# phecda-xu/FullyCNNSpeechEnhancement

Hardware: AMD Instinct MI355X
Metric: spectrogram frames/sec (CR-CED-16 fwd, 129-bin) (higher is better)
Workload: dtype f32; 1 GPU; CR-CED V3 (16-layer, skip connections) forward, batch 256 per GPU, 129x512, fp32 (BASELINE configs[2]); variant=FullyCNNV3, batch_per_gpu=256, frames=512, bins=129, global_batch=256, fused_available=True, parallelism=batch-shard x1, rccl_world_size=1, weights=random-init (glorot, seed 42), library=rced-hip 0.1 gfx950

## Files before the change

fullycnnspeechenhancement_amd/csrc/kernels_fused_v3.h:

```cpp
#pragma once
#include <hip/hip_runtime.h>

#include <type_traits>

#include "lds_dma.h"

#ifndef RCED_V3_LEGACY_FORMS
#define RCED_V3_LEGACY_FORMS 0
#endif
#ifndef RCED_D1
#define RCED_D1 1
#endif
#ifndef RCED_D2
#define RCED_D2 2
#endif
#ifndef RCED_D2X
#define RCED_D2X 1
#endif
#ifndef RCED_D3
#define RCED_D3 2
#endif
#ifndef RCED_LANE_OPAQUE
#define RCED_LANE_OPAQUE 1
#endif
#ifndef RCED_L1_ORDER
#define RCED_L1_ORDER 1
#endif
#ifndef RCED_L3_CHAINS
#define RCED_L3_CHAINS 2
#endif
#ifndef RCED_L2_BOTH
#define RCED_L2_BOTH 1
#endif
#ifndef RCED_T_L1X6
#define RCED_T_L1X6 1
#endif
#ifndef RCED_T_L1SWAP
#define RCED_T_L1SWAP 1
#endif
#ifndef RCED_V3_LB
#define RCED_V3_LB kThreads
#endif
#ifndef RCED_STAMPS
#define RCED_STAMPS 0
#endif

namespace rced {
namespace v3 {

#if RCED_STAMPS
__device__ __forceinline__ unsigned long long stamp() {
  unsigned long long t;
  __builtin_amdgcn_sched_barrier(0);
  asm volatile("s_memtime %0\n\ts_waitcnt lgkmcnt(0)" : "=s"(t)::"memory");
  __builtin_amdgcn_sched_barrier(0);
  return t;
}
#define STAMP_BEGIN() const unsigned long long st_a_ = stamp()
#define STAMP_MATH(i) const unsigned long long st_b_ = stamp(); tsum[i] += st_b_ - st_a_
#define STAMP_WAIT(i) tsum[(i) + ((i) < 3 ? 3 : 1)] += stamp() - st_b_
#define DET_ARG , unsigned long long (&td)[16]
#define DET_PASS , tdet
#define DET_BEGIN() unsigned long long dt_ = stamp()
#define DET(k) do { const unsigned long long n_ = stamp(); td[k] += n_ - dt_; dt_ = n_; } while (0)
#if RCED_STAMPS == 2
#define DETX(k) DET(8 + (k))
#else
#define DETX(k)
#endif
#else
#define DETX(k)
#define STAMP_BEGIN()
#define STAMP_MATH(i)
#define STAMP_WAIT(i)
// ... 112 lines not shown
static_assert(kG1 % 4 == 0 && kG2 % 4 == 0 && kW3 % 4 == 0, "16-byte aligned pieces");
static_assert(kW1 + kFin128 <= kWRegion && (kW1 % 4) == 0, "F32 form: the bin-128 weights fit behind a layer-1 packet in its LDS region");

constexpr int kL3MT = 5;
constexpr int kW3TData = kL3MT * 3 * 256;
constexpr int kW3T = kW3TData + kShiftPerLayer;
constexpr int kTBlock = kG1 + kG2 + kW3T;
constexpr int kG1XMain = 9 * 256, kG1XRem = 12 * 256;
constexpr int kG1X = kG1XMain + kG1XRem + kShiftPerLayer;
constexpr int kTBlockX = kG1X + kG2 + kW3T;
constexpr int kTTotal = RCED_T_L1X6 ? kTBlock + 4 * kTBlockX : 5 * kTBlock;
constexpr int kB8PlaneBytes = kB8Rows * 16;
static_assert(kW3T % 4 == 0 && kG2 + kW3T <= 2 * kWRegion, "layer 3's fused-form packet: 16-byte pieces, inside a weight region");
#if RCED_V3_LEGACY_FORMS
#include "kernels_fused_v3_legacy_map.h"
#endif
constexpr int kHFr = 140;
constexpr int kHRows = kTF * kHFr;
constexpr int kHPlaneBytes = kHRows * 16;
constexpr int kHZeroRow = kHRows - 1;
constexpr int kFinTRows = 160;
constexpr int kFinTPart = kFinTRows * 16;
constexpr int kFinTFloats = 3 * kFinTPart / 4;
constexpr int kG1AMain = 8 * 256;
constexpr int kG1A = kG1AMain + kG1XRem + kShiftPerLayer;
constexpr int kG1APieces = (kG1AMain + kG1XRem) / 256;
constexpr int kTBlockA = kG1A + kG2 + kW3T;
constexpr int kATotal = 5 * kTBlockA;
template <>
struct Map<3> {
  static constexpr bool X6 = true, kX6 = true, kFused = true, kAllX6 = true, kL1X6 = true;
  static_assert(RCED_T_L1X6 != 0, "the all-x6 form is built on layer1_x6l");
  static constexpr int kB8Off = 0;
  static constexpr int kB8RegionBytes = 3 * (kHPlaneBytes > kB8PlaneBytes ? kHPlaneBytes : kB8PlaneBytes);
  static constexpr int kB18Off = kB8Off + kB8RegionBytes / 4;
  static constexpr int kHalfBytes = ((kB18Rows * 16 + 255) / 256) * 256;
  static constexpr int kRemOff = 2 * kHalfBytes;
  static constexpr int kRemRows = kB18Rows + 6;
  static constexpr int kPlaneBytes = ((kRemOff + kRemRows * 4 + 15) / 16) * 16;
  static constexpr int kRemHMBytes = 0, kRemLBytes = 0;
  static constexpr int kB18Bytes = 3 * kPlaneBytes;
  static constexpr int kWOff = kB18Off + kB18Bytes / 4;
  static constexpr int kW3TOff = kWOff + kG2;
  static constexpr int kWRegions = 1;
  static constexpr int kB30Off = kWOff;
  static constexpr int kW1Off = kW3TOff + kW3T;
  static constexpr int kFinTOff = kW1Off + kG1A;
  static constexpr int kX0Off = kFinTOff + kFinTFloats;
  static constexpr int kHOff = kB8Off, kFin128Off = kB8Off;
  static constexpr int kEdgeOff = kX0Off + kX0Floats;
  static constexpr int kEdgeFlagOff = kEdgeOff + 4 * 2 * 128;
  static constexpr int kTailOff = kEdgeFlagOff + 8;
  static constexpr int kTailFloats = (2 * 3 * 16 * 8 + 4 * 5 * 4 * 8 + 16) / 4;
  static constexpr int kLdsFloats = kTailOff + kTailFloats;
  static constexpr int kLdsBytes = kLdsFloats * 4;
  static_assert(kLdsBytes <= 160 * 1024, "LDS budget");
  static_assert((kB18Off * 4) % 16 == 0 && (kWOff * 4) % 16 == 0 && (kW3TOff * 4) % 16 == 0 && (kW1Off * 4) % 16 == 0 && (kFinTOff * 4) % 16 == 0 &&
                (kX0Off * 4) % 16 == 0 && (kEdgeOff * 4) % 16 == 0, "aligned buffers");
  static constexpr int finscr(int w, int ct) { return kB18Off * 4 + ct * kPlaneBytes + (w >> 2) * kHalfBytes + (kB18Pad + kS * (w & 3)) * 16; }
  static constexpr int kT1R = 128 * kB8S * 4, kT1W = 128 * 16;
  static constexpr int kT2R = 0, kT2W = 0, kT3R = 0, kT3W = 0;
  static constexpr int kTileB18 = 16 * 16;
};
typedef Map<3> MapA;
static_assert(MapA::finscr(7, 2) % 16 == 0 && MapA::finscr(3, 0) + 1024 <= MapA::kB18Off * 4 + (kB18Pad + kS * 3 + kF) * 16, "partial sums: aligned, inside real rows");


// ... 173 lines not shown
    L.wr1rl = PL + M::kRemLBytes + (rpx + 2 * kq + kB18Pad) * 4;
    if constexpr (M::kFused) L.wr1r = PL + M::kRemOff + (rpx + 2 * kq + kB18Pad) * 4;
    const int px2 = M::kFused ? kS * (wave & 3) + 64 * (wave >> 2) + n : RCED_L2_BOTH ? px0 : 16 * (wave & 3) + n;
    L.rd2m = PL + (px2 + (kq >> 1)) * 32 + (kq & 1) * 16;
    if constexpr (M::kAllX6) L.rd2m = PL + (kq & 1) * M::kHalfBytes + (px2 + (kq >> 1)) * 16;
    L.rd2r = PL + M::kRemHMBytes + (px2 + 4 * (kq & 1)) * 8;
    L.rd2rl = PL + M::kRemLBytes + (px2 + 4 * (kq & 1)) * 4;
    if constexpr (M::kFused) {
      L.rd2c = kq < 2 ? L.rd2m + (M::kAllX6 ? 64 : 128) : PL + M::kRemOff + (px2 + 4 * (kq & 1)) * 4;
      L.rd2cs = kq < 2 ? (unsigned)M::kTileB18 : 64u;
      asm volatile("" : "+v"(L.rd2c), "+v"(L.rd2cs));
    }
    L.rd2 = L.rd2b = L.rd2t = L.rd2tb = 0u;
  } else {
    const unsigned B18 = lds_addr(lds + M::kB18Off + kB18Pad * 18);
    L.wr1 = B18 + 4 * (px0 * 18 + 4 * kq);
    L.wr1r = B18 + 4 * ((rpx + 2 * kq) * 18 + 16);
    L.rd2 = B18 + 4 * ((px0 - 2) * 18 + 2 * kq);
    L.rd2t = L.rd2 + 4 * (8 * kL2Steps + (kq < 1 ? kq : 1) - 2 * kq);
    L.wr1rl = L.rd2m = L.rd2r = L.rd2rl = 0u;
  }
  if constexpr (M::kX6 && !RCED_L2_BOTH) L.wr2 = B30 + 4 * ((16 * (wave & 3) + n) * 30 + 16 * (wave >> 2) + 4 * kq);
  else L.wr2 = B30 + 4 * (px0 * 30 + 4 * kq);
  L.rd3 = B30 + 4 * ((2 * px0 - 4) * 30 + 2 * kq);
  L.rd3t = L.rd3 + 4 * (8 * kL3Steps - kq);
  L.wr3 = B8 + 4 * ((2 * px0 + (kq >> 1)) * kB8S + 4 * (kq & 1));
  if constexpr (M::kFused) L.wr3 = B8 + 4 * ((kS * (wave & 3) + 64 * (wave >> 2) + n) * kB8S + 2 * kq);
  if constexpr (M::kFused) {
    const unsigned B8P = lds_addr(lds + M::kB8Off);
    L.rd1x = B8P + (px0 - 4 + kq + kB8Pad) * 16;
    L.rd1xb = L.rd1x + 128 * 16;
    L.rd1xr = B8P + (rpx - 4 + kq + kB8Pad) * 16;
    L.wr3p = B8P + (kS * (wave & 3) + 64 * (wave >> 2) + n + kB8Pad) * 16 + 4 * kq;
    L.rd1f = L.rd1x + (8 - kq) * 16 + (kq < 2 ? 0 : kq - 1) * kB8PlaneBytes;
    asm volatile("" : "+v"(L.rd1x), "+v"(L.rd1xb), "+v"(L.rd1xr), "+v"(L.wr3p), "+v"(L.rd1f));
  }
  {
    const unsigned H = lds_addr(lds + M::kHOff);
    auto haddr = [&](int px) {
      const int fr = px / kS, f = px - fr * kS;
      return H + 4 * ((kHFrame * fr + 64 + f) * kHS + 4 * (kq & 1));
    };
    L.wh0 = haddr(2 * px0 + (kq >> 1));
    L.wh1 = haddr(2 * (px0 + 128) + (kq >> 1));
    L.whx = haddr(2 * (256 + n) + (kq >> 1));
    if constexpr (M::kFused) L.wh0 = H + 4 * ((kHFrame * (wave & 3) + 64 + 64 * (wave >> 2) + n) * kHS + 2 * kq);
    if constexpr (M::kAllX6) L.wh0 = lds_addr(lds + M::kB8Off) + (kHFr * (wave & 3) + 68 * (wave >> 2) + n) * 16 + 4 * kq;
  }
  unsigned v = 0;
#pragma unroll
  for (int t = 0; t < 4; ++t) v |= (unsigned)px_valid(px0 + 128 * t) << (kVMain + t);
#pragma unroll
  for (int r = 0; r < 2; ++r) {
    const int p = kRemPx * (16 * (r == 0 ? xr0 : 4) + nr) + 2 * kq;
    v |= (unsigned)(p >= 0 && px_valid(p)) << (kVRem + 2 * r);
    v |= (unsigned)(p >= 0 && px_valid(p + 1) && 2 * kq + 1 < kRemPx) << (kVRem + 2 * r + 1);
  }
#pragma unroll
  for (int t = 0; t < 2; ++t) v |= (unsigned)px_valid(2 * (px0 + 128 * t) + (kq >> 1)) << (kVL3 + t);
  v |= (unsigned)px_valid(2 * (256 + n) + (kq >> 1)) << kVL3X;
  v |= (unsigned)(lane < 48) << kVLt48;
  v |= (unsigned)(lane >= 32) << kVUpper;
  v |= (unsigned)(n == 0) << kVN0;
  if constexpr (M::kX6) {
    v |= (unsigned)(wave < 4 || lane < 48) << kVSt2;
#pragma unroll
    for (int t = 0; t < 8; ++t) v |= (unsigned)px_valid(16 * (wave & 3) + n + 64 * t) << (kVL2 + t);
// ... 966 lines not shown
          if constexpr (kL1X) a1x_dma<M>(wsrc + (M::kAllX6 ? kTBlockA : blk == 0 ? kTBlock : kTBlockX), lds, wave, lane);
        };
        layer23<M, false>(P, L, lds0, lds_addr(WREG(0)), A2, blk, wave, 0x80000000u | epoch, sk1, sk2, sp, dma1 DET_PASS);
        STAMP_MATH(2);
        layer_end_sync();
        STAMP_WAIT(2);
      } else {
        STAMP_BEGIN();
        const unsigned wb = lds_addr(WREG(M::kX6 ? 0 : wcur));
        ++epoch;
        const unsigned tag = 0x80000000u | epoch;
        const float* wnext = wsrc + kBlockFloats;
        auto dma = [&] {
          if constexpr (!M::kX6) packet_dma<kW1>(wnext, WREG(wcur ^ 1), wave, lane);
        };
        const unsigned voff = (unsigned)opaque(lane) * 16u;
        auto sp = [&](auto kc) {
          if constexpr (M::kX6 && !(RCED_X6_EXP & 4) && decltype(kc)::value < 7) wload(kc, gofs + kBlockFloats, voff);
        };
        layer3<M, false>(P, L, lds0, wb, blk, wave, tag, skip_ce1, skip_ce2, dma, sp DET_PASS);
        if constexpr (!M::kX6) wcur ^= 1;
        STAMP_MATH(2);
        layer_end_sync();
        STAMP_WAIT(2);
      }
      wsrc += M::kAllX6 ? kTBlockA : kL1X && blk > 0 ? kTBlockX : kBlockFloats;
      gofs += M::kAllX6 ? kTBlockA : kL1X && blk > 0 ? kTBlockX : kBlockFloats;
    }
    FinA finA;
    if constexpr (M::kAllX6) {
      STAMP_BEGIN();
      ++epoch;
      xst = xstage_load(P, tile + 1 < tile_end ? tile + 1 : P.total_tiles, tid);
      if (wave == 0 && lane < 3) lds_st<u32x4>(lds0 + 4 * M::kB8Off + kHZeroRow * 16 + (unsigned)lane * kHPlaneBytes, 0, u32x4{0u, 0u, 0u, 0u});
      auto dma1 = [&] { a1x_dma<M>(P.wpack, lds, wave, lane); };
      layer23<M, true>(P, L, lds0, lds_addr(WREG(0)), A2, 4, wave, 0x80000000u | epoch, sk1, sk2, [](auto) {}, dma1 DET_PASS);
      STAMP_MATH(2);
      layer_end_sync();
      STAMP_WAIT(2);
    } else if constexpr (M::kFused) {
      STAMP_BEGIN();
      ++epoch;
      xst = xstage_load(P, tile + 1 < tile_end ? tile + 1 : P.total_tiles, tid);
      const int lane_o = opaque(lane);
      auto sp = [&](auto jc) {
        constexpr int j = decltype(jc)::value, s0 = (kFinRun * j) / 5, s1 = (kFinRun * (j + 1)) / 5;
        const f32x2* src = reinterpret_cast<const f32x2*>(P.fin) + (size_t)(kFinRun * wave) * 64 + lane_o;
#pragma unroll
        for (int q = s0; q < s1; ++q) finA.a[q] = src[q * 64];
      };
      layer23<M, true>(P, L, lds0, lds_addr(WREG(0)), A2, 4, wave, 0x80000000u | epoch, sk1, sk2, sp, [] {} DET_PASS);
      STAMP_MATH(2);
      layer_end_sync();
      STAMP_WAIT(2);
      const unsigned voff = (unsigned)opaque(lane) * 16u;
      static_for<0, 7>([&](auto kc) { wload(kc, 0, voff); });
    } else {
      STAMP_BEGIN();
      const unsigned wb = lds_addr(WREG(M::kX6 ? 0 : wcur));
      ++epoch;
      const unsigned tag = 0x80000000u | epoch;
      xst = xstage_load(P, tile + 1 < tile_end ? tile + 1 : P.total_tiles, tid);
      if constexpr (M::kX6) packet_dma<kFin128>(P.fin + kFinA, lds + M::kFin128Off, wave, lane);
      else packet_dma<kFin128>(P.fin + kFinA, WREG(wcur ^ 1) + kW1, wave, lane);
      fin_prefetch(P, wave, lane, finA);
      fin_zero_pads<M>(lds0, tid);
      auto dma = [&] {
        if constexpr (!M::kX6) packet_dma<kW1>(P.wpack, WREG(wcur ^ 1), wave, lane);
      };
      const unsigned voff = (unsigned)opaque(lane) * 16u;
      auto sp = [&](auto kc) {
        if constexpr (M::kX6 && !(RCED_X6_EXP & 4) && decltype(kc)::value < 7) wload(kc, 0, voff);
      };
      layer3<M, true>(P, L, lds0, wb, 4, wave, tag, skip_ce1, skip_ce2, dma, sp DET_PASS);
      if constexpr (!M::kX6) wcur ^= 1;
      STAMP_MATH(2);
      layer_end_sync();
      STAMP_WAIT(2);
    }
#if RCED_STAMPS
    const unsigned long long st_f_ = stamp();
#endif
    if constexpr (M::kAllX6) {
      final_phase_x6<M>(P, lds0, wave, lane, utt, t0, xst, lds + M::kX0Off DET_PASS);
    } else {
      const unsigned w128 = M::kX6 ? lds0 + 4 * M::kFin128Off : lds_addr(WREG(wcur) + kW1);
      final_phase<M>(P, lds0, w128, wave, lane, utt, t0, finA, xst, lds + M::kX0Off);
    }
#if RCED_STAMPS
    tfin += stamp() - st_f_;
#endif
  }
#undef WREG
#if RCED_STAMPS
  if (P.stamps && blockIdx.x == 0 && lane == 0)
    for (int i = 0; i < 8; ++i) P.stamps[wave * 8 + i] = tsum[i];
  if (P.stamps && blockIdx.x == 0 && lane == 0) P.stamps[64 + wave * 3] = tfin;
  if (P.stamps && blockIdx.x == 0 && lane == 0)
    for (int i = 0; i < 16; ++i) P.stamps[88 + wave * 16 + i] = tdet[i];
#endif
}


}
}
```

fullycnnspeechenhancement_amd/csrc/kernels_fused_v3_allx6.h:

```cpp
#pragma once

template <class M>
__device__ __forceinline__ void convert_px(unsigned lds0, int i, int f) {
  const unsigned src = lds0 + 4 * (M::kX0Off + 4 + i * kS + f);
  float v[8];
#pragma unroll
  for (int rr = 0; rr < 8; ++rr) v[rr] = lds_ld<float>(src, rr * kS * 4);
  u32x4 h, m, l;
#pragma unroll
  for (int q = 0; q < 4; ++q) {
    const P3 p = split2(v[2 * q], v[2 * q + 1]);
    h[q] = p.h;
    m[q] = p.m;
    l[q] = p.l;
  }
  const unsigned dst = lds0 + 4 * M::kB8Off + (kB8Pad + i * kS + f) * 16;
  lds_st<u32x4>(dst, 0, h);
  lds_st<u32x4>(dst, kB8PlaneBytes, m);
  lds_st<u32x4>(dst, 2 * kB8PlaneBytes, l);
}
template <class M>
__device__ __forceinline__ void convert_x0(unsigned lds0, int wave, int lane) {
  lane = opaque(lane);
  const int tid = wave * 64 + lane;
  convert_px<M>(lds0, tid >> 7, tid & 127);
  if (wave == 7 && lane < kTF) convert_px<M>(lds0, lane, kF - 1);
  const int z = tid - 5 * 64;
  if (z >= 0 && z < 72) {
    const int part = z / 24, rr = z - part * 24;
    const int row = rr < 4 ? rr : rr < 20 ? kB8Pad + kS * ((rr - 4) >> 2) + kF + ((rr - 4) & 3) : kB8Pad + kNPX + (rr - 20);
    lds_st<u32x4>(lds0 + 4 * M::kB8Off + part * kB8PlaneBytes + row * 16, 0, u32x4{0u, 0u, 0u, 0u});
  }
}
static_assert(kB8Rows == kB8Pad + kNPX + 4, "convert_x0 zeroes the planes' pad, gap and trailing rows by this map");

template <class M, int NCH, bool CT2ALL>
__device__ __forceinline__ void fin_run(unsigned ra, unsigned ta, int b0, int b2, int q0, bool ct2first, unsigned zaddr, f32x4 (&acc)[3]) {
  s16x8 a[2][3];
  Parts b[2][3];
  auto ld = [&](auto ic) {
    constexpr int i = decltype(ic)::value, r = i & 1;
    const int q = q0 + i;
    const unsigned ta_i = ta + (unsigned)(64 * q);
#pragma unroll
    for (int p = 0; p < 3; ++p) a[r][p] = lds_ld<s16x8>(ta_i, p * kFinTPart);
    const unsigned ra_i = ra + (unsigned)(16 * (4 * q + (q >> 2)));
    const int bq = b0 + 4 * q;
#pragma unroll
    for (int ct = 0; ct < 3; ++ct) {
      if (ct == 2 && !(CT2ALL || i == 0)) continue;
      const bool ok = ct < 2 ? (unsigned)(bq + 64 * ct) <= 128u : (unsigned)(b2 + 4 * q) <= 128u;
      const unsigned ad = ok ? ra_i + 1088u * ct : zaddr;
      b[r][ct].h = lds_ld<s16x8>(ad, 0);
      b[r][ct].m = lds_ld<s16x8>(ad, kHPlaneBytes);
      b[r][ct].l = lds_ld<s16x8>(ad, 2 * kHPlaneBytes);
    }
  };
  ld(IC<0>{});
  pin();
  static_for<0, NCH>([&](auto ic) {
    constexpr int i = decltype(ic)::value, r = i & 1;
    if constexpr (i + 1 < NCH) ld(IC<i + 1>{});
    pin();
    mma2(a[r], b[r][0], acc[0], a[r], b[r][1], acc[1]);
    if constexpr (CT2ALL) {
      acc[2] = l2x_mma(a[r], b[r][2], acc[2]);
    } else if constexpr (i == 0) {
      if (ct2first) acc[2] = l2x_mma(a[r], b[r][2], acc[2]);
    }
    pin();
  });
}

template <class M>
__device__ __forceinline__ void final_phase_x6(const Params& P, unsigned lds0, int wave, int lane, int utt, int t0, const XStage& xnext, float* x0 DET_ARG) {
  DET_BEGIN();
  lane = opaque(lane);
  const int n = lane & 15, kq = lane >> 4;
  const f32x4 zero4 = {0.f, 0.f, 0.f, 0.f};
  float* yt = P.y + ((size_t)utt * P.T + t0) * kF;
  const int nfr = P.T - t0 < kTF ? P.T - t0 : kTF;
  xstage_store(xnext, x0, wave * 64 + lane);
  {
    const int fi = n >> 2, j0 = n & 3;
    const int b0 = 16 * j0 - 64 + kq;
    const int b2 = j0 == 0 ? b0 + 128 : 0x40000000;
    const unsigned ra = lds0 + 4 * M::kB8Off + (unsigned)((kHFr * fi + 17 * j0 - 68 + kq) * 16);
    const unsigned ta = lds0 + 4 * M::kFinTOff + (unsigned)((kq - n + 15) * 16);
    const unsigned zaddr = lds0 + 4 * M::kB8Off + kHZeroRow * 16;
    f32x4 acc[3] = {zero4, zero4, zero4};
    if (wave < 4) {
      fin_run<M, 4, true>(ra, ta, b0, b2, 4 * wave, false, zaddr, acc);
    } else {
      const int run = 11 - wave;
      fin_run<M, 5, false>(ra, ta, b0, b2, 16 + 5 * (run - 4), run == 4, zaddr, acc);
    }
    const unsigned scr = lds0 + (unsigned)M::finscr(wave, 0) + (unsigned)lane * 16u;
#pragma unroll
    for (int ct = 0; ct < 3; ++ct) lds_st<f32x4>(scr, ct * M::kPlaneBytes, acc[ct]);
  }
  DET(8);
  __syncthreads();
  DET(9);
  if (wave < 3) {
    const unsigned scr = lds0 + (unsigned)(M::finscr(0, 0) + wave * M::kPlaneBytes) + (unsigned)lane * 16u;
    f32x4 v = lds_ld<f32x4>(scr, 0);
#pragma unroll
    for (int w = 1; w < kWaves; ++w) v += lds_ld<f32x4>(scr, M::finscr(w, 0) - M::finscr(0, 0));
    v += f32x4{P.fin_bias, P.fin_bias, P.fin_bias, P.fin_bias};
    const int fi = n >> 2;
    if (wave < 2) {
      const int f0 = 16 * (4 * wave + (n & 3)) + 4 * kq;
      if (fi < nfr) {
        *reinterpret_cast<f32x4_u*>(yt + fi * kF + f0) = v;
        store_wait_state();
      }
    } else if (kq == 0 && (n & 3) == 0 && fi < nfr) {
      yt[fi * kF + kF - 1] = v.x;
    }
  }
  DET(10);
  convert_x0<M>(lds0, wave, lane);
  DET(11);
  __syncthreads();
  DET(12);
}
```

fullycnnspeechenhancement_amd/csrc/kernels_fused_v3_l23.h:

```cpp
#pragma once
#ifndef RCED_T_A2REG
#define RCED_T_A2REG 3
#endif
#ifndef RCED_T_PRIO
#define RCED_T_PRIO 1
#endif
#ifndef RCED_T_TAILW
#define RCED_T_TAILW 4
#endif
#ifndef RCED_T_A3D
#define RCED_T_A3D 1
#endif
#ifndef RCED_T_SGB
#define RCED_T_SGB 1
#endif
#ifndef RCED_T_L1PF
#define RCED_T_L1PF 1
#endif
#ifndef RCED_T_EXP
#define RCED_T_EXP 0
#endif
#if (RCED_T_EXP != 0 || RCED_X6_EXP != 0) && !defined(RCED_TIMING_ONLY)
#error "RCED_T_EXP / RCED_X6_EXP builds compute wrong results: timing experiments only (tools/mkexp.sh ... -DRCED_TIMING_ONLY -DRCED_T_EXP=...)"
#endif
// ... 169 lines not shown
    bb.m = __builtin_bit_cast(s16x8, b3m[1]);
    bb.l = __builtin_bit_cast(s16x8, b3l[1]);
    f32x4 ca = zero4, cb = zero4;
    mma2(a3r[r], ba, ca, a3r[r], bb, cb);
    if constexpr (j == kL3MT - 1) {
      p4[0] = ca;
      p4[1] = cb;
    } else {
      pj[0][j & 1] = ca;
      pj[1][j & 1] = cb;
    }
  };
  auto finish = [&](auto tc, float s0, float s1) {
    constexpr int t = decltype(tc)::value;
    f32x2 v = {relu1(s0 + sh3.x), relu1(s1 + sh3.y)};
    if constexpr (LAST) {
      v += sk1[t];
    } else {
      v += blk == 3 ? sk2[t] : zero2;
      sk1[t] = blk == 0 ? v : sk1[t];
      sk2[t] = blk == 1 ? v : sk2[t];
    }
    if constexpr (M::kAllX6 && LAST) {
      const P3 p = split2(v.x, v.y);
      if (t < 4 || vbit(L, kVN0)) {
        lds_st<unsigned>(L.wh0, t * 272, p.h);
        lds_st<unsigned>(L.wh0, t * 272 + kHPlaneBytes, p.m);
        lds_st<unsigned>(L.wh0, t * 272 + 2 * kHPlaneBytes, p.l);
      }
    } else if constexpr (RCED_T_L1X6 && !LAST) {
      const P3 p = split2(v.x, v.y);
      if (t < 4 || vbit(L, kVN0)) {
        lds_st<unsigned>(L.wr3p, t * 256, p.h);
        lds_st<unsigned>(L.wr3p, t * 256 + kB8PlaneBytes, p.m);
        lds_st<unsigned>(L.wr3p, t * 256 + 2 * kB8PlaneBytes, p.l);
      }
    } else {
      if (t < 4 || vbit(L, kVN0)) lds_st<f32x2>(LAST ? L.wh0 : L.wr3, t * (16 * kB8S * 4), v);
    }
  };
  static_assert(kHS == kB8S, "one tile stride for both destinations");
  const unsigned edge = lds0 + 4 * M::kEdgeOff + fr * 1024 + L.a8, eflag = lds0 + 4 * M::kEdgeFlagOff + fr * 8;
  auto publish = [&](int dir, float v0, float v1) {
    lds_st<f32x2>(edge, dir * 512, f32x2{v0, v1});
    cbar();
    if (L.a4 == 0) lds_poke_a(eflag + dir * 4, tag);
  };
  auto fetch = [&](int dir) {
    flag_wait(eflag + dir * 4, tag, P.err, 8u);
    return lds_ld<f32x2>(edge, dir * 512);
  };
  auto tail_pair = [&](auto ac) {
    constexpr int a = decltype(ac)::value;
    shift_add<4>(p4[0], w0, w1, x0, x1, y0, y1);
    shift_add<4>(p4[1], x0, x1, y0, y1, z0, z1);
    if constexpr (a == 0) {
      if (right) {
        publish(1, w0, w1);
        hold = f32x2{x0, x1};
      } else {
        finish(IC<0>{}, x0, x1);
      }
    } else {
      finish(IC<a - 1>{}, w0, w1);
      finish(IC<a>{}, x0, x1);
    }
    w0 = y0;
    w1 = y1;
// ... 162 lines not shown
      const int ti = tn >= 12 ? 16 - tn : 0;
      const f32x2 r = lds_ld<f32x2>(tb + kT3 + (unsigned)((fr * 5 + ti) * 4 + tkq) * 8u, 0);
      if (tn >= 12) {
        w0 += r.x;
        w1 += r.y;
      } else if (tn == 0) {
        x0 += r.x;
        x1 += r.y;
      }
    }
    finish(i3, w0, w1);
    finish(i4, x0, x1);
    const f32x2 e = fetch(0);
    finish(i0, hold.x + e.x, hold.y + e.y);
    if (RCED_T_PRIO) __builtin_amdgcn_s_setprio(0);
  } else {
    runX(i3, i0, [&] { tail_pair(i0); });
    runX(i4, i1, none);
    DET(2);
    runY(i2, i1, i1, i0, i0, none);
    static_for<0, 4>([&](auto qc) { split_piece(i4, qc); });
    runY(i4, i0, i2, i0, IC<kL3MT % (RCED_T_A3D + 1)>{}, [&] { tail_pair(i2); });
    shift_add<4>(p4[0], w0, w1, x0, x1, y0, y1);
    finish(i3, w0, w1);
    finish(i4, x0, x1);
    const f32x2 e = fetch(0);
    finish(i0, hold.x + e.x, hold.y + e.y);
    if (RCED_T_PRIO) __builtin_amdgcn_s_setprio(0);
  }
  DET(3);
}


__device__ __forceinline__ Parts b8_load(unsigned rd, int off) {
  Parts b;
  b.h = lds_ld<s16x8>(rd, off);
  if (RCED_T_EXP & 256) {
    b.m = b.l = b.h;
    return b;
  }
  b.m = lds_ld<s16x8>(rd, off + kB8PlaneBytes);
  b.l = lds_ld<s16x8>(rd, off + 2 * kB8PlaneBytes);
  return b;
}

template <class M>
constexpr int a1x_off(int i) {
  if constexpr (M::kAllX6) return M::kW1Off * 4 + i * 1024;
  else return i < 5 ? M::kX0Off * 4 + i * 1024
                    : M::kHOff * 4 + (kHFrame * ((i - 5) / 4) + 64) * kHS * 4 + 8 * (((i - 5) / 4) & 1) + ((i - 5) % 4) * 1024;
}
template <class M>
constexpr int a1x_shift_off() {
  if constexpr (M::kAllX6) return M::kW1Off * 4 + kG1APieces * 1024;
  else return M::kX0Off * 4 + 5 * 1024;
}
#if RCED_V3_LEGACY_FORMS
static_assert(a1x_shift_off<MapT>() + 128 <= (MapT::kX0Off + kX0Floats) * 4 && a1x_off<MapT>(20) + 1024 <= (MapT::kHOff + (kHFrame * 3 + 64 + kF) * kHS) * 4 &&
              a1x_off<MapT>(8) % 16 == 0 && a1x_off<MapT>(9) % 16 == 0 && a1x_off<MapT>(13) % 16 == 0 && a1x_off<MapT>(17) % 16 == 0,
              "layer 1's LDS-resident images: inside the input-row area / the real bins of the H image, 16-byte aligned");
#endif
template <class M>
__device__ __forceinline__ void a1x_dma(const float* src, float* lds, int wave, int lane) {
  constexpr int kPieces = M::kAllX6 ? kG1APieces : 21;
  lane = opaque(lane);
#pragma unroll
  for (int k = 0; k < 3; ++k) {
    const int ci = wave + 8 * k;
    if (ci < kPieces) {
      lds_dma16s(src + ci * 256, (unsigned)lane * 16u, lds + a1x_off<M>(ci) / 4);
    } else if (ci == kPieces) {
      if (lane < 8) lds_dma16s(src + kPieces * 256, (unsigned)lane * 16u, lds + a1x_shift_off<M>() / 4);
    }
  }
}
template <class M, int I>
__device__ __forceinline__ s16x8 a1x_ld(unsigned aX, unsigned aH) {
  if constexpr (I < 5 || M::kAllX6) return lds_ld<s16x8>(aX, I * 1024);
  else return lds_ld<s16x8>(aH, a1x_off<M>(I) - M::kHOff * 4);
}
template <class M, class Dma, class Sp>
__device__ __forceinline__ void layer1_x6l(const Lane& L, unsigned lds0, int role, Dma dma, Sp sp DET_ARG) {
  DET_BEGIN();
  constexpr int kTW = M::kT1W, kTR = 128 * 16;
  const unsigned aX = lds0 + (M::kAllX6 ? a1x_off<M>(0) : M::kX0Off * 4) + L.scr, aH = lds0 + M::kHOff * 4 + L.scr;
  const f32x4 sh = lds_ld<f32x4>(lds0 + a1x_shift_off<M>() + L.kq16, 0);
  const f32x2 s2 = lds_ld<f32x2>(lds0 + a1x_shift_off<M>(), 64);
  auto pre = once(dma);
  auto lda = [&](auto pc, s16x8 (&a)[3]) {
    constexpr int g = decltype(pc)::value;
    a[0] = a1x_ld<M, 3 * g>(aX, aH);
    a[1] = a1x_ld<M, 3 * g + 1>(aX, aH);
    a[2] = a1x_ld<M, 3 * g + 2>(aX, aH);
  };
  constexpr bool kPF = M::kAllX6 && RCED_T_L1PF;
  constexpr bool kFold = M::kAllX6;
  constexpr int kRemPiece = kFold ? 8 : 9;
  auto ldar = [&](auto cc, s16x8 (&a)[3]) {
    constexpr int c = decltype(cc)::value;
    a[0] = a1x_ld<M, kRemPiece + 3 * c>(aX, aH);
    a[1] = a1x_ld<M, kRemPiece + 3 * c + 1>(aX, aH);
    a[2] = a1x_ld<M, kRemPiece + 3 * c + 2>(aX, aH);
  };
  const bool has_single = role < 2 || role == 7, has_rem = role >= 4;
  const unsigned rd_single = L.rd1x + (role == 0 ? 32 : role == 1 ? 30 : 16) * 256;
  Parts nb;
  s16x8 na[3];
  auto prefetch = [&](unsigned rd, int aoff) {
    nb = b8_load(rd, 0);
#pragma unroll
    for (int q = 0; q < 3; ++q) na[q] = lds_ld<s16x8>(aX + aoff, q * 1024);
  };
  if constexpr (kFold) {
    Parts b[2][2];
    s16x8 bf[2];
    s16x8 a[2][3], af[2];
    f32x4 acc[2][2];
    const bool two = role != 7;
    const bool g1 = tile_has_gap(role + 8), g2 = tile_has_gap(role + 16), g3 = tile_has_gap(role + 24);
    auto ld = [&](auto ic) {
      constexpr int i = decltype(ic)::value, p = i / 2, c = i % 2;
      if constexpr (p == 0) lda(IC<c>{}, a[c]);
      b[c][0] = b8_load(L.rd1x, 2 * p * kTR + 64 * c);
      b[c][1] = b8_load(L.rd1xb, 2 * p * kTR + 64 * c);
      if constexpr (c == 1) {
        if constexpr (p == 0) {
          af[0] = a1x_ld<M, 6>(aX, aH);
          af[1] = a1x_ld<M, 7>(aX, aH);
        }
        if (RCED_T_EXP & 32768) return;
        bf[0] = lds_ld<s16x8>(L.rd1f, 2 * p * kTR);
        bf[1] = lds_ld<s16x8>(L.rd1f, 2 * p * kTR + 128 * 16);
      }
    };
    auto slot = [&](auto ic) {
      constexpr int i = decltype(ic)::value, p = i / 2, c = i % 2;
      if constexpr (c == 0) acc[p][0] = acc[p][1] = sh;
      mma2(a[c], b[c][0], acc[p][0], a[c], b[c][1], acc[p][1]);
      if (c == 1 && !(RCED_T_EXP & 32768)) {
        acc[p][0] = mfma32(af[0], bf[0], acc[p][0]);
        acc[p][1] = mfma32(af[0], bf[1], acc[p][1]);
        acc[p][0] = mfma32(af[1], bf[0], acc[p][0]);
        acc[p][1] = mfma32(af[1], bf[1], acc[p][1]);
      }
      if constexpr (p == 0) static_for<0, (c == 0 ? 4 : 5)>([&](auto qc) { sp(IC<12 + 4 * c + decltype(qc)::value>{}); });
      if constexpr (i == 2) l1_store<M>(L, acc[0][0], L.wr1, 0, false, kVMain);
      if constexpr (i == 3) l1_store<M>(L, acc[0][1], L.wr1, kTW, g1, kVMain + 1);
      interleave<(c == 1 && !(RCED_T_EXP & 32768) ? 16 : 12), 3>();
    };
    ld(IC<0>{});
    pin();
    if (!(RCED_T_EXP & 512)) pre();
    pin();
    static_for<0, 2>([&](auto ic) {
      constexpr int i = decltype(ic)::value;
      if constexpr (i < 1) ld(IC<i + 1>{});
      else if (two) ld(IC<2>{});
// ... 6 lines not shown
      static_for<2, 4>([&](auto ic) {
        constexpr int i = decltype(ic)::value;
        if constexpr (i < 3) ld(IC<i + 1>{});
        pin();
        slot(ic);
        pin();
        DETX(i);
      });
      if constexpr (kPF) {
        if (has_single) prefetch(rd_single, 0);
        else if (has_rem) prefetch(L.rd1xr, kRemPiece * 1024);
        pin();
      }
      l1_store<M>(L, acc[1][0], L.wr1, 2 * kTW, g2, kVMain + 2);
      l1_store<M>(L, acc[1][1], L.wr1, 3 * kTW, g3, kVMain + 3);
      DETX(6);
    } else {
      if constexpr (kPF) {
        prefetch(rd_single, 0);
        pin();
      }
      l1_store<M>(L, acc[0][0], L.wr1, 0, false, 0);
      l1_store<M>(L, acc[0][1], L.wr1, kTW, false, 0);
    }
  } else {
    Parts b[2][2];
    s16x8 a[3][3];
    f32x4 acc[2][2];
    const bool two = role != 7;
    const bool g1 = tile_has_gap(role + 8), g2 = tile_has_gap(role + 16), g3 = tile_has_gap(role + 24);
    auto ld = [&](auto ic) {
      constexpr int i = decltype(ic)::value, p = i / 3, c = i % 3;
      if constexpr (p == 0) lda(IC<c>{}, a[c]);
      b[i & 1][0] = b8_load(L.rd1x, 2 * p * kTR + 64 * c);
      b[i & 1][1] = b8_load(L.rd1xb, 2 * p * kTR + 64 * c);
    };
    auto slot = [&](auto ic) {
      constexpr int i = decltype(ic)::value, p = i / 3, c = i % 3;
      if constexpr (c == 0) acc[p][0] = acc[p][1] = sh;
      mma2(a[c], b[i & 1][0], acc[p][0], a[c], b[i & 1][1], acc[p][1]);
      if constexpr (p == 0) static_for<0, 3>([&](auto qc) { sp(IC<12 + 3 * i + decltype(qc)::value>{}); });
      if constexpr (p == 1 && c == 0) l1_store<M>(L, acc[0][0], L.wr1, 0, false, kVMain);
      if constexpr (p == 1 && c == 1) l1_store<M>(L, acc[0][1], L.wr1, kTW, g1, kVMain + 1);
      interleave<12, 3>();
    };
    ld(IC<0>{});
    pin();
    if (!(RCED_T_EXP & 512)) pre();
    pin();
    static_for<0, 3>([&](auto ic) {
      constexpr int i = decltype(ic)::value;
      if constexpr (i < 2) ld(IC<i + 1>{});
      else if (two) ld(IC<3>{});
      pin();
      slot(ic);
      pin();
      DETX(i);
    });
    if (two) {
      static_for<3, 6>([&](auto ic) {
        constexpr int i = decltype(ic)::value;
        if constexpr (i < 5) ld(IC<i + 1>{});
        pin();
        slot(ic);
        pin();
        DETX(i);
      });
      if constexpr (kPF) {
        if (has_single) prefetch(rd_single, 0);
        else if (has_rem) prefetch(L.rd1xr, kRemPiece * 1024);
        pin();
      }
      l1_store<M>(L, acc[1][0], L.wr1, 2 * kTW, g2, kVMain + 2);
      l1_store<M>(L, acc[1][1], L.wr1, 3 * kTW, g3, kVMain + 3);
      DETX(6);
    } else {
      if constexpr (kPF) {
        prefetch(rd_single, 0);
        pin();
      }
      l1_store<M>(L, acc[0][0], L.wr1, 0, false, 0);
      l1_store<M>(L, acc[0][1], L.wr1, kTW, false, 0);
    }
  }
  DET(6);
  if (RCED_T_EXP & 8192) return;
  if (role < 2 || role == 7) {
    const int dt = role == 0 ? 32 : role == 1 ? 30 : 16;
    const unsigned rd = L.rd1x + dt * 256;
    Parts b[2];
    s16x8 a[2][3];
    f32x4 acc = sh;
    if constexpr (kPF) {
      b[0] = nb;
      a[0][0] = na[0];
      a[0][1] = na[1];
      a[0][2] = na[2];
    } else {
      b[0] = b8_load(rd, 0);
      lda(IC<0>{}, a[0]);
    }
    pin();
    static_for<0, 3>([&](auto cc) {
      constexpr int c = decltype(cc)::value;
      if constexpr (kFold && c == 1) {
        if (!(RCED_T_EXP & 32768)) b[0].h = lds_ld<s16x8>(L.rd1f + dt * 256, 0);
        a[0][0] = a1x_ld<M, 6>(aX, aH);
        a[0][1] = a1x_ld<M, 7>(aX, aH);
      } else if constexpr (c < 2) {
        b[(c + 1) & 1] = b8_load(rd, 64 * (c + 1));
        lda(IC<c + 1>{}, a[(c + 1) & 1]);
      }
      pin();
      if ((RCED_T_EXP & 32768) && c == 2) {
      } else if constexpr (kFold && c == 2) {
        acc = mfma32(a[0][0], b[0].h, acc);
        acc = mfma32(a[0][1], b[0].h, acc);
      } else {
        acc = l2x_mma(a[c & 1], b[c & 1], acc);
      }
      pin();
    });
    if constexpr (kPF) {
      if (has_rem) prefetch(L.rd1xr, kRemPiece * 1024);
      pin();
    }
    l1_store<M>(L, acc, L.wr1 + dt * M::kTileB18, 0, false, 0);
  }
  DET(5);
  {
    const int nrem = role < 4 ? 0 : role == 7 ? 2 : 1;
    unsigned rdr = L.rd1xr, wrr = L.wr1r;
    int xr = role == 7 ? 3 : role - 4, vb = kVRem;
    const f32x4 init = {s2.x, s2.y, s2.x, s2.y};
#pragma unroll 1
    for (int r = 0; r < nrem; ++r) {
      Parts b[2];
      s16x8 a[2][3];
      f32x4 acc = init;
      if (kPF && r == 0) {
        b[0] = nb;
        a[0][0] = na[0];
        a[0][1] = na[1];
        a[0][2] = na[2];
      } else {
        b[0] = b8_load(rdr, 0);
        ldar(IC<0>{}, a[0]);
      }
      pin();
      static_for<0, 4>([&](auto cc) {
        constexpr int c = decltype(cc)::value;
        if constexpr (c < 3) {
          b[(c + 1) & 1] = b8_load(rdr, 64 * (c + 1));
          ldar(IC<c + 1>{}, a[(c + 1) & 1]);
        }
        pin();
        acc = l2x_mma(a[c & 1], b[c & 1], acc);
        pin();
      });
      const f32x4 v = relu4(acc);
      const bool va = xr == 0 || vbit(L, vb), vbb = vbit(L, vb + 1);
      const P3 pa = split2(v.x, v.y), pb = split2(v.z, v.w);
      if (va) {
        lds_st<unsigned>(wrr, 0, pa.h);
        lds_st<unsigned>(wrr, M::kPlaneBytes, pa.m);
        lds_st<unsigned>(wrr, 2 * M::kPlaneBytes, pa.l);
      }
      if (vbb) {
        lds_st<unsigned>(wrr, 4, pb.h);
        lds_st<unsigned>(wrr, M::kPlaneBytes + 4, pb.m);
        lds_st<unsigned>(wrr, 2 * M::kPlaneBytes + 4, pb.l);
      }
      wrr += 112 * 4;
      rdr += 112 * 16;
      xr += 1;
      vb += 2;
    }
  }
  DET(4);
}
```

fullycnnspeechenhancement_amd/csrc/kernels_fused_v3_legacy_map.h:

```cpp
#pragma once
template <>
struct Map<2> {
  static constexpr bool X6 = true, kX6 = true, kFused = true, kAllX6 = false;
  static constexpr int kB8Off = 0;
  static constexpr bool kL1X6 = RCED_T_L1X6 != 0;
  static constexpr int kB18Off = kB8Off + (kL1X6 ? 3 * kB8PlaneBytes / 4 : kB8Rows * kB8S);
  static constexpr int kRemOff = kB18Rows * 32;
  static constexpr int kRemRows = kB18Rows + 6;
  static constexpr int kPlaneBytes = ((kRemOff + kRemRows * 4 + 15) / 16) * 16;
  static constexpr int kRemHMBytes = 0, kRemLBytes = 0;
  static constexpr int kB18Bytes = 3 * kPlaneBytes;
  static constexpr int kWOff = kB18Off + kB18Bytes / 4;
  static constexpr int kW3TOff = kWOff + kG2;
  static constexpr int kWRegions = 1;
  static constexpr int kB30Off = kWOff;
  static constexpr int kX0Off = kW3TOff + kW3T;
  static constexpr int kHOff = kX0Off + kX0Floats;
  static constexpr int kFin128Off = kHOff + kHPix * kHS;
  static constexpr int kEdgeOff = kFin128Off + kFin128;
  static constexpr int kEdgeFlagOff = kEdgeOff + 4 * 2 * 128;
  static constexpr int kLdsFloats = kEdgeFlagOff + 8;
  static constexpr int kLdsBytes = kLdsFloats * 4;
  static_assert(kLdsBytes <= 160 * 1024, "LDS budget");
  static_assert((kWOff * 4) % 16 == 0 && (kW3TOff * 4) % 16 == 0 && (kB18Off * 4) % 16 == 0 && (kHOff % 2) == 0, "aligned buffers");
  static_assert((kFin128Off * 4) % 16 == 0 && (kEdgeOff * 4) % 16 == 0, "aligned buffers");
  static constexpr int finscr0(int w) {
    return kL1X6 ? kB8Off * 4 + (w >> 2) * kB8PlaneBytes + (kB8Pad + kS * (w & 3)) * 16
                 : (kB8Off + (kB8Pad + kS * (w >> 1)) * kB8S) * 4 + 8 * ((w >> 1) & 1) + (w & 1) * 2048;
  }
  static constexpr int kFinScrCt = 1024;
  static constexpr int kT1R = 128 * kB8S * 4, kT1W = 128 * 32;
  static constexpr int kT2R = 0, kT2W = 0, kT3R = 0, kT3W = 0;
  static constexpr int kTileB18 = 16 * 32;
};
typedef Map<2> MapT;
static_assert(MapT::finscr0(7) % 16 == 0 && MapT::finscr0(2) % 16 == 0 && (MapT::kL1X6 || MapT::finscr0(1) + 2048 <= (kB8Pad + kF) * kB8S * 4), "decode_final's partial sums: 16-byte aligned, inside real rows of B8");

// ... 2 lines not shown
```

Measured before the change: 23.07 million frames/s.

## Overlap next-tile input conversion with final layer MMAs and widen B8 plane stride

The next tile's input staging store moves to the end of the layer2/3 phase. The fp32-to-split-bf16 conversion of the next tile's input now runs inside the final-layer MMA loop: reads come first, the splits are interleaved with MMA slots, and the stores happen after the barrier. Before, the conversion ran serially after the final reduction. The B8 plane stride is widened to the H plane size (a multiple of 256 bytes), which removes the separate zero-row store and is meant to keep the rd1f lane groups free of bank conflicts. The final cross-wave partial-sum loads are batched before they are summed. The cost is more live registers during the final phase and a larger LDS region.

Measured after the change: 23.21 million frames/s (median of 6 runs). No clear change (+0.6%).

```diff
diff --git a/fullycnnspeechenhancement_amd/csrc/kernels_fused_v3.h b/fullycnnspeechenhancement_amd/csrc/kernels_fused_v3.h
--- a/fullycnnspeechenhancement_amd/csrc/kernels_fused_v3.h
+++ b/fullycnnspeechenhancement_amd/csrc/kernels_fused_v3.h
@@ -40,6 +40,9 @@
 #endif
 #ifndef RCED_V3_LB
 #define RCED_V3_LB kThreads
+#endif
+#ifndef RCED_T_B8STRIDE
+#define RCED_T_B8STRIDE 1
 #endif
 #ifndef RCED_STAMPS
 #define RCED_STAMPS 0
@@ -218,7 +221,9 @@
   static constexpr bool X6 = true, kX6 = true, kFused = true, kAllX6 = true, kL1X6 = true;
   static_assert(RCED_T_L1X6 != 0, "the all-x6 form is built on layer1_x6l");
   static constexpr int kB8Off = 0;
-  static constexpr int kB8RegionBytes = 3 * (kHPlaneBytes > kB8PlaneBytes ? kHPlaneBytes : kB8PlaneBytes);
+  static constexpr int kB8Plane = RCED_T_B8STRIDE ? kHPlaneBytes : kB8PlaneBytes;
+  static_assert(kB8Plane >= kB8PlaneBytes && kB8Plane % 16 == 0 && (!RCED_T_B8STRIDE || kB8Plane % 256 == 0), "the planes fit their stride; lane groups of rd1f stay conflict-free");
+  static constexpr int kB8RegionBytes = 3 * (kHPlaneBytes > kB8Plane ? kHPlaneBytes : kB8Plane);
   static constexpr int kB18Off = kB8Off + kB8RegionBytes / 4;
   static constexpr int kHalfBytes = ((kB18Rows * 16 + 255) / 256) * 256;
   static constexpr int kRemOff = 2 * kHalfBytes;
@@ -458,7 +463,7 @@
     L.rd1xb = L.rd1x + 128 * 16;
     L.rd1xr = B8P + (rpx - 4 + kq + kB8Pad) * 16;
     L.wr3p = B8P + (kS * (wave & 3) + 64 * (wave >> 2) + n + kB8Pad) * 16 + 4 * kq;
-    L.rd1f = L.rd1x + (8 - kq) * 16 + (kq < 2 ? 0 : kq - 1) * kB8PlaneBytes;
+    L.rd1f = L.rd1x + (8 - kq) * 16 + (kq < 2 ? 0 : kq - 1) * M::kB8Plane;
     asm volatile("" : "+v"(L.rd1x), "+v"(L.rd1xb), "+v"(L.rd1xr), "+v"(L.wr3p), "+v"(L.rd1f));
   }
   {
@@ -1491,9 +1496,12 @@
       STAMP_BEGIN();
       ++epoch;
       xst = xstage_load(P, tile + 1 < tile_end ? tile + 1 : P.total_tiles, tid);
-      if (wave == 0 && lane < 3) lds_st<u32x4>(lds0 + 4 * M::kB8Off + kHZeroRow * 16 + (unsigned)lane * kHPlaneBytes, 0, u32x4{0u, 0u, 0u, 0u});
+      if constexpr (M::kB8Plane != kHPlaneBytes) {
+        if (wave == 0 && lane < 3) lds_st<u32x4>(lds0 + 4 * M::kB8Off + kHZeroRow * 16 + (unsigned)lane * kHPlaneBytes, 0, u32x4{0u, 0u, 0u, 0u});
+      }
       auto dma1 = [&] { a1x_dma<M>(P.wpack, lds, wave, lane); };
       layer23<M, true>(P, L, lds0, lds_addr(WREG(0)), A2, 4, wave, 0x80000000u | epoch, sk1, sk2, [](auto) {}, dma1 DET_PASS);
+      xstage_store(xst, lds + M::kX0Off, tid);
       STAMP_MATH(2);
       layer_end_sync();
       STAMP_WAIT(2);
@@ -1541,7 +1549,7 @@
     const unsigned long long st_f_ = stamp();
 #endif
     if constexpr (M::kAllX6) {
-      final_phase_x6<M>(P, lds0, wave, lane, utt, t0, xst, lds + M::kX0Off DET_PASS);
+      final_phase_x6<M>(P, lds0, wave, lane, utt, t0 DET_PASS);
     } else {
       const unsigned w128 = M::kX6 ? lds0 + 4 * M::kFin128Off : lds_addr(WREG(wcur) + kW1);
       final_phase<M>(P, lds0, w128, wave, lane, utt, t0, finA, xst, lds + M::kX0Off);
diff --git a/fullycnnspeechenhancement_amd/csrc/kernels_fused_v3_allx6.h b/fullycnnspeechenhancement_amd/csrc/kernels_fused_v3_allx6.h
--- a/fullycnnspeechenhancement_amd/csrc/kernels_fused_v3_allx6.h
+++ b/fullycnnspeechenhancement_amd/csrc/kernels_fused_v3_allx6.h
@@ -1,41 +1,59 @@
 #pragma once
 
+struct CvPx {
+  float v[8];
+  u32x4 h, m, l;
+};
 template <class M>
-__device__ __forceinline__ void convert_px(unsigned lds0, int i, int f) {
+__device__ __forceinline__ void cv_read(unsigned lds0, int i, int f, CvPx& c) {
   const unsigned src = lds0 + 4 * (M::kX0Off + 4 + i * kS + f);
-  float v[8];
 #pragma unroll
-  for (int rr = 0; rr < 8; ++rr) v[rr] = lds_ld<float>(src, rr * kS * 4);
-  u32x4 h, m, l;
-#pragma unroll
-  for (int q = 0; q < 4; ++q) {
-    const P3 p = split2(v[2 * q], v[2 * q + 1]);
-    h[q] = p.h;
-    m[q] = p.m;
-    l[q] = p.l;
+  for (int rr = 0; rr < 8; ++rr) c.v[rr] = lds_ld<float>(src, rr * kS * 4);
+}
+template <int Q>
+__device__ __forceinline__ void cv_split(CvPx& c) {
+  const P3 p = split2(c.v[2 * Q], c.v[2 * Q + 1]);
+  c.h[Q] = p.h;
+  c.m[Q] = p.m;
+  c.l[Q] = p.l;
+}
+template <class M>
+__device__ __forceinline__ void cv_store(unsigned lds0, int i, int f, const CvPx& c) {
+  const unsigned dst = lds0 + 4 * M::kB8Off + (kB8Pad + i * kS + f) * 16;
+  lds_st<u32x4>(dst, 0, c.h);
+  lds_st<u32x4>(dst, M::kB8Plane, c.m);
+  lds_st<u32x4>(dst, 2 * M::kB8Plane, c.l);
+}
+template <class M>
+__device__ __forceinline__ void cv_zero_rows(unsigned lds0, int tid) {
+  constexpr int kRows = 4 + 4 * (kTF - 1) + (M::kB8Plane / 16 - kB8Pad - kNPX + 4);
+  static_assert(kB8Rows == kB8Pad + kNPX + 4 && kS - kF == 4 && 3 * kRows <= 3 * 64 && kB8Pad + kNPX - 4 + (kRows - 16) == M::kB8Plane / 16,
+                "the planes' pad and gap rows and everything behind the last frame's bins, one store per thread of waves 5..7");
+  const int z = tid - 5 * 64;
+  if (z >= 0 && z < 3 * kRows) {
+    const int part = z / kRows, rr = z - part * kRows;
+    const int row = rr < 4 ? rr : rr < 16 ? kB8Pad + kS * ((rr - 4) >> 2) + kF + ((rr - 4) & 3) : kB8Pad + kNPX - 4 + (rr - 16);
+    lds_st<u32x4>(lds0 + 4 * M::kB8Off + part * M::kB8Plane + row * 16, 0, u32x4{0u, 0u, 0u, 0u});
   }
-  const unsigned dst = lds0 + 4 * M::kB8Off + (kB8Pad + i * kS + f) * 16;
-  lds_st<u32x4>(dst, 0, h);
-  lds_st<u32x4>(dst, kB8PlaneBytes, m);
-  lds_st<u32x4>(dst, 2 * kB8PlaneBytes, l);
 }
 template <class M>
 __device__ __forceinline__ void convert_x0(unsigned lds0, int wave, int lane) {
   lane = opaque(lane);
   const int tid = wave * 64 + lane;
-  convert_px<M>(lds0, tid >> 7, tid & 127);
-  if (wave == 7 && lane < kTF) convert_px<M>(lds0, lane, kF - 1);
-  const int z = tid - 5 * 64;
-  if (z >= 0 && z < 72) {
-    const int part = z / 24, rr = z - part * 24;
-    const int row = rr < 4 ? rr : rr < 20 ? kB8Pad + kS * ((rr - 4) >> 2) + kF + ((rr - 4) & 3) : kB8Pad + kNPX + (rr - 20);
-    lds_st<u32x4>(lds0 + 4 * M::kB8Off + part * kB8PlaneBytes + row * 16, 0, u32x4{0u, 0u, 0u, 0u});
+  CvPx c;
+  cv_read<M>(lds0, tid >> 7, tid & 127, c);
+  static_for<0, 4>([&](auto qc) { cv_split<decltype(qc)::value>(c); });
+  cv_store<M>(lds0, tid >> 7, tid & 127, c);
+  if (wave == 7 && lane < kTF) {
+    cv_read<M>(lds0, lane, kF - 1, c);
+    static_for<0, 4>([&](auto qc) { cv_split<decltype(qc)::value>(c); });
+    cv_store<M>(lds0, lane, kF - 1, c);
   }
+  cv_zero_rows<M>(lds0, tid);
 }
-static_assert(kB8Rows == kB8Pad + kNPX + 4, "convert_x0 zeroes the planes' pad, gap and trailing rows by this map");
 
-template <class M, int NCH, bool CT2ALL>
-__device__ __forceinline__ void fin_run(unsigned ra, unsigned ta, int b0, int b2, int q0, bool ct2first, unsigned zaddr, f32x4 (&acc)[3]) {
+template <class M, int NCH, bool CT2ALL, class Cv>
+__device__ __forceinline__ void fin_run(unsigned ra, unsigned ta, int b0, int b2, int q0, bool ct2first, unsigned zaddr, f32x4 (&acc)[3], Cv cv) {
   s16x8 a[2][3];
   Parts b[2][3];
   auto ld = [&](auto ic) {
@@ -68,19 +86,25 @@
     } else if constexpr (i == 0) {
       if (ct2first) acc[2] = l2x_mma(a[r], b[r][2], acc[2]);
     }
+    if constexpr (CT2ALL || i > 0) {
+      cv(ic);
+      interleave<(CT2ALL ? 18 : 12), 2>();
+    }
     pin();
   });
 }
 
 template <class M>
-__device__ __forceinline__ void final_phase_x6(const Params& P, unsigned lds0, int wave, int lane, int utt, int t0, const XStage& xnext, float* x0 DET_ARG) {
+__device__ __forceinline__ void final_phase_x6(const Params& P, unsigned lds0, int wave, int lane, int utt, int t0 DET_ARG) {
   DET_BEGIN();
   lane = opaque(lane);
   const int n = lane & 15, kq = lane >> 4;
   const f32x4 zero4 = {0.f, 0.f, 0.f, 0.f};
   float* yt = P.y + ((size_t)utt * P.T + t0) * kF;
   const int nfr = P.T - t0 < kTF ? P.T - t0 : kTF;
-  xstage_store(xnext, x0, wave * 64 + lane);
+  const int tid = wave * 64 + lane;
+  CvPx cva, cvb;
+  cv_read<M>(lds0, tid >> 7, tid & 127, cva);
   {
     const int fi = n >> 2, j0 = n & 3;
     const int b0 = 16 * j0 - 64 + kq;
@@ -90,10 +114,26 @@
     const unsigned zaddr = lds0 + 4 * M::kB8Off + kHZeroRow * 16;
     f32x4 acc[3] = {zero4, zero4, zero4};
     if (wave < 4) {
-      fin_run<M, 4, true>(ra, ta, b0, b2, 4 * wave, false, zaddr, acc);
+      fin_run<M, 4, true>(ra, ta, b0, b2, 4 * wave, false, zaddr, acc, [&](auto ic) {
+        constexpr int i = decltype(ic)::value;
+        if constexpr (i < 2) {
+          cv_split<2 * i>(cva);
+          cv_split<2 * i + 1>(cva);
+        }
+      });
     } else {
+      cv_read<M>(lds0, lane & (kTF - 1), kF - 1, cvb);
       const int run = 11 - wave;
-      fin_run<M, 5, false>(ra, ta, b0, b2, 16 + 5 * (run - 4), run == 4, zaddr, acc);
+      fin_run<M, 5, false>(ra, ta, b0, b2, 16 + 5 * (run - 4), run == 4, zaddr, acc, [&](auto ic) {
+        constexpr int i = decltype(ic)::value;
+        if constexpr (i == 1 || i == 2) {
+          cv_split<2 * i - 2>(cva);
+          cv_split<2 * i - 1>(cva);
+        } else if constexpr (i >= 3) {
+          cv_split<2 * i - 6>(cvb);
+          cv_split<2 * i - 5>(cvb);
+        }
+      });
     }
     const unsigned scr = lds0 + (unsigned)M::finscr(wave, 0) + (unsigned)lane * 16u;
 #pragma unroll
@@ -102,11 +142,19 @@
   DET(8);
   __syncthreads();
   DET(9);
+  cv_store<M>(lds0, tid >> 7, tid & 127, cva);
+  if (wave == 7 && lane < kTF) cv_store<M>(lds0, lane, kF - 1, cvb);
+  cv_zero_rows<M>(lds0, tid);
+  DET(11);
   if (wave < 3) {
     const unsigned scr = lds0 + (unsigned)(M::finscr(0, 0) + wave * M::kPlaneBytes) + (unsigned)lane * 16u;
-    f32x4 v = lds_ld<f32x4>(scr, 0);
+    f32x4 ps[kWaves];
 #pragma unroll
-    for (int w = 1; w < kWaves; ++w) v += lds_ld<f32x4>(scr, M::finscr(w, 0) - M::finscr(0, 0));
+    for (int w = 0; w < kWaves; ++w) ps[w] = lds_ld<f32x4>(scr, M::finscr(w, 0) - M::finscr(0, 0));
+    pin();
+    f32x4 v = ps[0];
+#pragma unroll
+    for (int w = 1; w < kWaves; ++w) v += ps[w];
     v += f32x4{P.fin_bias, P.fin_bias, P.fin_bias, P.fin_bias};
     const int fi = n >> 2;
     if (wave < 2) {
@@ -120,8 +168,6 @@
     }
   }
   DET(10);
-  convert_x0<M>(lds0, wave, lane);
-  DET(11);
   __syncthreads();
   DET(12);
 }
diff --git a/fullycnnspeechenhancement_amd/csrc/kernels_fused_v3_l23.h b/fullycnnspeechenhancement_amd/csrc/kernels_fused_v3_l23.h
--- a/fullycnnspeechenhancement_amd/csrc/kernels_fused_v3_l23.h
+++ b/fullycnnspeechenhancement_amd/csrc/kernels_fused_v3_l23.h
@@ -225,8 +225,8 @@
       const P3 p = split2(v.x, v.y);
       if (t < 4 || vbit(L, kVN0)) {
         lds_st<unsigned>(L.wr3p, t * 256, p.h);
-        lds_st<unsigned>(L.wr3p, t * 256 + kB8PlaneBytes, p.m);
-        lds_st<unsigned>(L.wr3p, t * 256 + 2 * kB8PlaneBytes, p.l);
+        lds_st<unsigned>(L.wr3p, t * 256 + M::kB8Plane, p.m);
+        lds_st<unsigned>(L.wr3p, t * 256 + 2 * M::kB8Plane, p.l);
       }
     } else {
       if (t < 4 || vbit(L, kVN0)) lds_st<f32x2>(LAST ? L.wh0 : L.wr3, t * (16 * kB8S * 4), v);
@@ -455,6 +455,7 @@
 }
 
 
+template <class M>
 __device__ __forceinline__ Parts b8_load(unsigned rd, int off) {
   Parts b;
   b.h = lds_ld<s16x8>(rd, off);
@@ -462,8 +463,8 @@
     b.m = b.l = b.h;
     return b;
   }
-  b.m = lds_ld<s16x8>(rd, off + kB8PlaneBytes);
-  b.l = lds_ld<s16x8>(rd, off + 2 * kB8PlaneBytes);
+  b.m = lds_ld<s16x8>(rd, off + M::kB8Plane);
+  b.l = lds_ld<s16x8>(rd, off + 2 * M::kB8Plane);
   return b;
 }
 
@@ -530,7 +531,7 @@
   Parts nb;
   s16x8 na[3];
   auto prefetch = [&](unsigned rd, int aoff) {
-    nb = b8_load(rd, 0);
+    nb = b8_load<M>(rd, 0);
 #pragma unroll
     for (int q = 0; q < 3; ++q) na[q] = lds_ld<s16x8>(aX + aoff, q * 1024);
   };
@@ -544,8 +545,8 @@
     auto ld = [&](auto ic) {
       constexpr int i = decltype(ic)::value, p = i / 2, c = i % 2;
       if constexpr (p == 0) lda(IC<c>{}, a[c]);
-      b[c][0] = b8_load(L.rd1x, 2 * p * kTR + 64 * c);
-      b[c][1] = b8_load(L.rd1xb, 2 * p * kTR + 64 * c);
+      b[c][0] = b8_load<M>(L.rd1x, 2 * p * kTR + 64 * c);
+      b[c][1] = b8_load<M>(L.rd1xb, 2 * p * kTR + 64 * c);
       if constexpr (c == 1) {
         if constexpr (p == 0) {
           af[0] = a1x_ld<M, 6>(aX, aH);
@@ -618,8 +619,8 @@
     auto ld = [&](auto ic) {
       constexpr int i = decltype(ic)::value, p = i / 3, c = i % 3;
       if constexpr (p == 0) lda(IC<c>{}, a[c]);
-      b[i & 1][0] = b8_load(L.rd1x, 2 * p * kTR + 64 * c);
-      b[i & 1][1] = b8_load(L.rd1xb, 2 * p * kTR + 64 * c);
+      b[i & 1][0] = b8_load<M>(L.rd1x, 2 * p * kTR + 64 * c);
+      b[i & 1][1] = b8_load<M>(L.rd1xb, 2 * p * kTR + 64 * c);
     };
     auto slot = [&](auto ic) {
       constexpr int i = decltype(ic)::value, p = i / 3, c = i % 3;
@@ -683,7 +684,7 @@
       a[0][1] = na[1];
       a[0][2] = na[2];
     } else {
-      b[0] = b8_load(rd, 0);
+      b[0] = b8_load<M>(rd, 0);
       lda(IC<0>{}, a[0]);
     }
     pin();
@@ -694,7 +695,7 @@
         a[0][0] = a1x_ld<M, 6>(aX, aH);
         a[0][1] = a1x_ld<M, 7>(aX, aH);
       } else if constexpr (c < 2) {
-        b[(c + 1) & 1] = b8_load(rd, 64 * (c + 1));
+        b[(c + 1) & 1] = b8_load<M>(rd, 64 * (c + 1));
         lda(IC<c + 1>{}, a[(c + 1) & 1]);
       }
       pin();
@@ -730,14 +731,14 @@
         a[0][1] = na[1];
         a[0][2] = na[2];
       } else {
-        b[0] = b8_load(rdr, 0);
+        b[0] = b8_load<M>(rdr, 0);
         ldar(IC<0>{}, a[0]);
       }
       pin();
       static_for<0, 4>([&](auto cc) {
         constexpr int c = decltype(cc)::value;
         if constexpr (c < 3) {
-          b[(c + 1) & 1] = b8_load(rdr, 64 * (c + 1));
+          b[(c + 1) & 1] = b8_load<M>(rdr, 64 * (c + 1));
           ldar(IC<c + 1>{}, a[(c + 1) & 1]);
         }
         pin();
diff --git a/fullycnnspeechenhancement_amd/csrc/kernels_fused_v3_legacy_map.h b/fullycnnspeechenhancement_amd/csrc/kernels_fused_v3_legacy_map.h
--- a/fullycnnspeechenhancement_amd/csrc/kernels_fused_v3_legacy_map.h
+++ b/fullycnnspeechenhancement_amd/csrc/kernels_fused_v3_legacy_map.h
@@ -3,6 +3,7 @@
 struct Map<2> {
   static constexpr bool X6 = true, kX6 = true, kFused = true, kAllX6 = false;
   static constexpr int kB8Off = 0;
+  static constexpr int kB8Plane = kB8PlaneBytes;
   static constexpr bool kL1X6 = RCED_T_L1X6 != 0;
   static constexpr int kB18Off = kB8Off + (kL1X6 ? 3 * kB8PlaneBytes / 4 : kB8Rows * kB8S);
   static constexpr int kRemOff = kB18Rows * 32;
```
